# HiromasaYamanishi/furusato_recommend

Hardware: AMD Instinct MI355X
Metric: BPR positive-edges/sec (LightGCN-3 d=64, 1000000 x 100000 / 20000000 edges) (higher is better)
Workload: dtype f32; 1 GPU; C2: LightGCN 3-layer d=64, synthetic 1000000 users x 100000 items / 20000000 edges (uniform); users=1000000, items=100000, edges=20000000, graph=uniform, dim=64, layers=3, bpr_batch_per_rank=2048, global_batch=2048, ranks=1, parallelism=dp1 (user-sharded, RCCL none gradient exchange)

## Files before the change

### furusato_recommend_amd/_lib.py

```python
from __future__ import annotations

import ctypes
import os
from ctypes import (POINTER, Structure, c_float, c_int, c_int32, c_int64,
                    c_size_t, c_uint64, c_void_p, c_char_p)

import torch

_HERE = os.path.dirname(os.path.abspath(__file__))
LIB_PATH = os.environ.get("MIREC_LIB") or os.path.join(_HERE, "libmirec.so")

MIREC_OK = 0
ERR_WORKSPACE = 4
ERR_RANGE = 5
IN_PRESCALED, IN_RAW, IN_SPARSE, IN_NONE = 0, 1, 2, 3
SUPPORTED_DIMS = (4, 8, 16, 32, 64, 128, 256)


class MirecError(RuntimeError):
    pass


class CSR(Structure):
    _fields_ = [
# ... 93 lines not shown
    "mirec_csr_long_rows": (c_int, [c_void_p, c_int64, c_int32, POINTER(c_int64),
                                    POINTER(c_int64), c_void_p, c_void_p, c_void_p,
                                    c_void_p]),
    "mirec_propagate": (c_int, [POINTER(CSR), POINTER(Prop), c_void_p]),
    "mirec_propagate_sweep": (c_int, [POINTER(CSR), POINTER(Prop), POINTER(Sweep), c_void_p]),
    "mirec_sweep_sizeof": (c_size_t, []),
    "mirec_sweep_shape": (c_int, [c_int64, c_int32, c_int32, POINTER(c_int32),
                                  POINTER(c_int32)]),
    "mirec_sweep_build": (c_int, [c_void_p, c_void_p, c_int64, c_int64, c_int64, c_int32,
                                  c_int32, c_void_p, c_void_p]),
    "mirec_sweep_groups": (c_int, [c_int32]),
    "mirec_sweep_wave_sizeof": (c_size_t, []),
    "mirec_sweep_wave_build": (c_int, [c_void_p, c_void_p, c_int64, c_int64, c_int64, c_int64,
                                       c_int32, c_void_p, c_void_p, c_int64, POINTER(c_int64)]),
    "mirec_sweep_wave_pack": (c_int, [c_void_p, c_int64, c_int64, c_int64, c_int32, c_void_p,
                                      POINTER(c_int32)]),
    "mirec_propagate_sweep_wave": (c_int, [POINTER(CSR), POINTER(Prop), POINTER(SweepWave),
                                           POINTER(SweepWave), c_void_p]),
    "mirec_sweep_pace_sizeof": (c_size_t, []),
    "mirec_sweep_pace_ws_bytes": (c_size_t, []),
    "mirec_propagate_sweep_wave_paced": (c_int, [POINTER(CSR), POINTER(Prop), POINTER(SweepWave),
                                                 POINTER(SweepWave), POINTER(SweepPace),
                                                 c_void_p]),
    "mirec_sweep_wave_stamp": (c_int, [POINTER(CSR), POINTER(Prop), POINTER(SweepWave), c_void_p,
                                       c_int64, c_void_p, c_void_p]),
    "mirec_drop_sizeof": (c_size_t, []),
    "mirec_propagate_drop": (c_int, [POINTER(CSR), POINTER(Prop), POINTER(Drop), c_void_p]),
    "mirec_edge_keep_mask": (c_int, [c_void_p, c_void_p, c_int64, c_uint64, c_float, c_int32,
                                     c_void_p]),
    "mirec_edge_dot": (c_int, [POINTER(CSR), c_void_p, c_void_p, c_int32, c_void_p, c_void_p]),
    "mirec_prescale": (c_int, [c_void_p, c_void_p, c_int64, c_int32, c_void_p, c_void_p]),
    "mirec_shard_pack": (c_int, [c_void_p, c_int64, c_int32, c_int32, c_int32, c_int64, c_int64,
                                 c_void_p, c_void_p]),
    "mirec_shard_unpack": (c_int, [c_void_p, c_int64, c_int32, c_int32, c_int32, c_int64,
                                   c_int64, c_void_p, c_void_p, c_void_p, c_void_p]),
    "mirec_frontier": (c_int, [POINTER(CSR), c_void_p, c_int64, c_void_p, c_void_p, c_void_p,
                               c_int64, c_int64, c_void_p, c_void_p, c_void_p, c_void_p,
                               c_void_p, c_int32, c_void_p]),
    "mirec_seed_bits_sizeof": (c_size_t, []),
    "mirec_frontier_bits": (c_int, [POINTER(CSR), c_void_p, c_int64, c_void_p, c_void_p, c_void_p,
                                    c_int64, c_int64, c_void_p, c_void_p, c_void_p, c_void_p,
                                    c_void_p, c_int32, POINTER(SeedBits), c_void_p]),
    "mirec_propagate_seeded": (c_int, [POINTER(CSR), POINTER(Prop), POINTER(SeedBits), c_void_p]),
    "mirec_mask_compact_pair": (c_int, [c_void_p, c_void_p, c_void_p, c_int64, c_void_p, c_void_p,
                                        c_void_p, c_void_p, c_void_p, c_void_p]),
    "mirec_small_sort_workspace": (c_int, [c_int64, POINTER(c_size_t)]),
# ... 346 lines not shown
```

### furusato_recommend_amd/csrc/prop.hip

```cpp
#include <mutex>
#include <set>
#include <type_traits>
#include <utility>

#include "common.h"

namespace mirec {

struct PropK {
  const int64_t *rowptr;
  const int32_t *col;
  const float *dinv;
  int64_t n_rows;
  int64_t n_seg;
  const int32_t *seg_row;
  const int64_t *seg_beg;
  int32_t split;
  const float *x_in;
  const int32_t *slot;
  const float *seed_in;
  const float *seed;
  const float *addend;
  const float *seed2;
  float divisor;
// ... 662 lines not shown
constexpr int kPaceMaxNaps = 8;
constexpr int kPaceMaxNapUnits = 16;
constexpr int kXccIdReg = 20 | (3 << 11);

struct SweepAuxK {
  unsigned *ws;
  int32_t lead;
  int32_t every;
  int32_t nap;
  long long *stamps;
  int32_t *meta;
};

__device__ __forceinline__ unsigned pace_read(const unsigned *p) {
  unsigned v;
  asm volatile("s_load_dword %0, %1, 0x0 glc\n\ts_waitcnt lgkmcnt(0)"
               : "=&s"(v)
               : "s"(p)
               : "memory");
  return v;
}

template <int D, int U, bool SCALED, int AUX = kAuxNone, bool PACKED = false,
          bool STREAM = false>
__device__ __forceinline__ void sweep_wave_work(const PropK &a, const SweepWaveK &s,
                                                const SweepAuxK &x = SweepAuxK{}) {
  constexpr int LPR = D / 4;
  constexpr int G = 64 / LPR;
  constexpr int NB = 64 / (U * G);
  static_assert(G == 4 && U * G == MIREC_SWEEP_BATCH && kSweepThreads / 64 == MIREC_SWEEP_WAVES,
                "the host layout's steps, batches and waves");
  extern __shared__ float4 sweep_acc[];
  const int lane = threadIdx.x & 63;
  const int sub = lane % LPR;
  const int g = lane / LPR;
  const int wid = __builtin_amdgcn_readfirstlane(threadIdx.x >> 6);
  using Slot = typename std::conditional<PACKED, unsigned, long long>::type;
  const Slot *slots = reinterpret_cast<const Slot *>(s.slot);
  [[maybe_unused]] const int col_bits = 32 - s.row_bits;
  const Slot kPadRow = PACKED ? (Slot)(~0u << col_bits) : (Slot)0xffffffff00000000ull;
  const int64_t last = s.n_slots - 1;
  int adv = 0, told = 0, due = 0;
  unsigned *pace_reg = nullptr, *pace_sum = nullptr;
  if constexpr (AUX == kAuxPace) {
    const int label = (int)__builtin_amdgcn_s_getreg(kXccIdReg) & (kPaceLabels - 1);
    pace_reg = x.ws + (2 * label) * kPaceLineWords;
    pace_sum = pace_reg + kPaceLineWords;
    due = x.every;
    if (wid == 0 && lane == 0)
      (void)__hip_atomic_fetch_add(pace_reg, 1u, __ATOMIC_RELAXED, __HIP_MEMORY_SCOPE_AGENT);
  }
  auto pace = [&]() {
    if constexpr (AUX == kAuxPace) {
      if (wid != 0) return;
      ++adv;
      if (--due != 0) return;
      due = x.every;
      if (lane == 0)
        (void)__hip_atomic_fetch_add(pace_sum, (unsigned)(adv - told), __ATOMIC_RELAXED,
                                     __HIP_MEMORY_SCOPE_AGENT);
      told = adv;
#pragma unroll 1
      for (int i = 0; i < kPaceMaxNaps; ++i) {
        const long long sum = pace_read(pace_sum), reg = pace_read(pace_reg);
// ... 4 lines not shown
    }
  };
  [[maybe_unused]] long long *stamp_lds = nullptr;
  if constexpr (AUX == kAuxStamp)
    stamp_lds = reinterpret_cast<long long *>(sweep_acc + (int64_t)s.tile_rows * LPR);
  auto stamp = [&](int i) {
    if constexpr (AUX == kAuxStamp) {
      if (wid == 0 && lane == 0) stamp_lds[i] = (long long)wall_clock64();
    }
  };
#pragma unroll 1
  for (int tile = blockIdx.x; tile < s.n_tiles; tile += gridDim.x) {
    stamp(0);
    const int64_t tile_row0 = (int64_t)tile * s.tile_rows;
    const int tile_len = (int)min((int64_t)s.tile_rows, s.n_rows - tile_row0);
    const int lr0 = min(wid * s.wave_rows, tile_len);
    const int lr1 = min(lr0 + s.wave_rows, tile_len);
    for (int lr = lr0 + g; lr < lr1; lr += G) sweep_acc[lr * LPR + sub] = f4_zero();
    int64_t pos = s.wptr[(int64_t)tile * MIREC_SWEEP_WAVES + wid];
    const int64_t end = s.wptr[(int64_t)tile * MIREC_SWEEP_WAVES + wid + 1];
    const int n_batches = __builtin_amdgcn_readfirstlane((int)((end - pos) / (U * G)));
    Slot cur = __builtin_nontemporal_load(slots + min(pos + lane, last));
    if (lane >= n_batches * (U * G)) cur |= kPadRow;
    int band = 0;
    int64_t hi = s.src0 + s.band_rows;
    float4 pv[U];
    int pr[U];
#pragma unroll
    for (int u = 0; u < U; ++u) {
      pv[u] = f4_zero();
      pr[u] = -1;
    }
#pragma unroll 1
    for (int b0 = 0; b0 < n_batches; b0 += NB) {
      Slot nxt = __builtin_nontemporal_load(slots + min(pos + 64 + lane, last));
      if (b0 * (U * G) + 64 + lane >= n_batches * (U * G)) nxt |= kPadRow;
      int ccol, crow;
      if constexpr (PACKED) {
        ccol = (int)s.src0 + (int)(cur & ~kPadRow);
        crow = cur >= kPadRow ? -1 : (int)(cur >> col_bits);
      } else {
        ccol = (int)(cur & 0xffffffffll);
        crow = (int)(cur >> 32);
      }
#pragma unroll
      for (int k = 0; k < NB; ++k) {
        const int nc = __builtin_amdgcn_readlane(ccol, k * U * G);
        while (b0 + k < n_batches && band + 1 < s.n_bands && (int64_t)nc >= hi) {
          pace();
          __builtin_amdgcn_s_barrier();
          ++band;
          hi += s.band_rows;
          stamp(band);
        }
        float4 v[U];
        int r[U];
#pragma unroll
        for (int u = 0; u < U; ++u) {
          const int src = k * U * G + u * G + g;
          const int j = __shfl(ccol, src);
          r[u] = __shfl(crow, src);
          v[u] = ld4(a.x_in + (int64_t)j * D + sub * 4);
        }
#pragma unroll
        for (int u = 0; u < U; ++u) {
          if (pr[u] >= 0) {
            float4 *p = &sweep_acc[pr[u] * LPR + sub];
            *p = f4_add(*p, pv[u]);
          }
        }
#pragma unroll
        for (int u = 0; u < U; ++u) {
          pv[u] = v[u];
          pr[u] = r[u];
        }
      }
      pos += 64;
      cur = nxt;
    }
    while (band + 1 < s.n_bands) {
      pace();
      __builtin_amdgcn_s_barrier();
      ++band;
      stamp(band);
    }
#pragma unroll
    for (int u = 0; u < U; ++u) {
      if (pr[u] >= 0) {
        float4 *p = &sweep_acc[pr[u] * LPR + sub];
        *p = f4_add(*p, pv[u]);
      }
    }
    for (int lr = lr0 + g; lr < lr1; lr += G)
      row_epilogue<D, SCALED, STREAM>(a, s.row0 + tile_row0 + lr, sweep_acc[lr * LPR + sub],
                                      sub);
    if constexpr (AUX == kAuxStamp) {
      stamp(s.n_bands);
      if (wid == 0) {
        long long *o = x.stamps + (int64_t)tile * (s.n_bands + 1);
        for (int b = lane; b <= s.n_bands; b += 64) o[b] = stamp_lds[b];
        if (lane == 0) {
// ... 12 lines not shown
      asm volatile("s_waitcnt vmcnt(0)" ::: "memory");
      unsigned *done = x.ws + 2 * kPaceLabels * kPaceLineWords;
      const unsigned left = __hip_atomic_fetch_add(done, 1u, __ATOMIC_RELAXED,
                                                   __HIP_MEMORY_SCOPE_AGENT);
      if (left == gridDim.x - 1) {
        for (int i = 0; i <= 2 * kPaceLabels; ++i)
          __hip_atomic_store(x.ws + i * kPaceLineWords, 0u, __ATOMIC_RELAXED,
                             __HIP_MEMORY_SCOPE_AGENT);
      }
    }
  }
}

template <int D, int U, bool SCALED, bool PACKED = false, bool STREAM = false>
__global__ __launch_bounds__(kSweepThreads) __attribute__((amdgpu_waves_per_eu(4, 4)))
MIREC_NO_PK_F32 void prop_sweep_wave_kernel(PropK a, SweepWaveK s) {
  sweep_wave_work<D, U, SCALED, kAuxNone, PACKED, STREAM>(a, s);
}

template <int D, int U, bool SCALED, int AUX, bool PACKED = false, bool STREAM = false>
__global__ __launch_bounds__(kSweepThreads) __attribute__((amdgpu_waves_per_eu(4, 4)))
MIREC_NO_PK_F32 void prop_sweep_wave_aux_kernel(PropK a, SweepWaveK s, SweepAuxK x) {
  sweep_wave_work<D, U, SCALED, AUX, PACKED, STREAM>(a, s, x);
}

using PropFn = void (*)(PropK);

template <int D, int UNROLL>
static PropFn prop_kernel_for(int mode, bool masked, bool rowmask, bool weighted, bool scaled,
                              bool dropout) {
  if (mode == MIREC_IN_SPARSE) masked = true;
  if (mode == MIREC_IN_NONE) weighted = dropout = false;
#define MIREC_PROP_CASE(MODE_W, MASKED)                               \
  case (MODE_W) * 2 + (MASKED):                                       \
    return rowmask ? prop_kernel<D, UNROLL, (MODE_W), MASKED, true>   \
                   : prop_kernel<D, UNROLL, (MODE_W), MASKED, false>;
  switch ((mode | (weighted ? kWeighted : 0) | (scaled ? kScaled : 0) |
           (dropout ? kDropout : 0)) * 2 + masked) {
    MIREC_PROP_CASE(MIREC_IN_PRESCALED | kWeighted, false)
    MIREC_PROP_CASE(MIREC_IN_PRESCALED, false)
    MIREC_PROP_CASE(MIREC_IN_PRESCALED | kWeighted, true)
    MIREC_PROP_CASE(MIREC_IN_PRESCALED, true)
    MIREC_PROP_CASE(MIREC_IN_RAW | kWeighted, false)
    MIREC_PROP_CASE(MIREC_IN_RAW, false)
    MIREC_PROP_CASE(MIREC_IN_RAW | kWeighted, true)
    MIREC_PROP_CASE(MIREC_IN_RAW, true)
// ... 145 lines not shown
      }
#pragma unroll
      for (int u = 0; u < UNROLL; ++u) {
        const float d = group_sum<LPR>(f4_dot(va[u], vb[u]));
        const float t = __shfl(d, (lane & (G - 1)) * LPR);
        if (lane >= k + u * G && lane < k + (u + 1) * G) res = t;
      }
    }
    if (lane < cnt) out[base + lane] = res;
  }
}

template <int D, int UNROLL>
static int launch_edge_dot(const mirec_csr_t *c, const float *a, const float *b, float *out,
                           hipStream_t st) {
  const int64_t waves = (c->nnz + kDotChunk - 1) / kDotChunk;
  const int64_t blocks = (waves + kWavesPerBlock - 1) / kWavesPerBlock;
  hipLaunchKernelGGL((edge_dot_kernel<D, UNROLL>), dim3((unsigned)blocks), dim3(256), 0, st,
                     c->rowptr, c->col, c->n_rows, c->nnz, a, b, out);
  MIREC_LAUNCH_CHECK();
  return MIREC_OK;
}

static bool sweep_launch_qualifies(const mirec_csr_t *c, const mirec_prop_t *p) {
  if (p->dim != 64) return false;
  if (c->val != nullptr) return false;
  if (p->in_mode != MIREC_IN_PRESCALED) return false;
  if (p->in_mask != nullptr || p->row_mask != nullptr || p->row_list != nullptr) return false;
  return c->n_seg == 0;
}

static bool sweep_qualifies(const mirec_csr_t *c, const mirec_prop_t *p, const mirec_sweep_t *sw) {
  if (sw == nullptr || !sweep_launch_qualifies(c, p)) return false;
  if (sw->gptr == nullptr || sw->ent == nullptr || sw->n_rows <= 0 || sw->n_tiles <= 0)
    return false;
  if (sw->row0 < 0 || sw->row0 + sw->n_rows != c->n_rows || sw->n_src > c->n_rows) return false;
  if (sw->tile_rows <= 0 || sw->group_rows <= 0 || sw->band_rows <= 0) return false;
  if (sw->groups <= 0 || sw->groups > kSweepThreads / (64 / 4)) return false;
  if ((int64_t)sw->groups * sw->group_rows < sw->tile_rows) return false;
  if ((int64_t)sw->n_tiles * sw->tile_rows < sw->n_rows) return false;
  if ((int64_t)sw->tile_rows * 64 * 4 > kSweepLdsDefault) return false;
  return true;
}

template <int D, int UNROLL>
static int launch_head(const mirec_csr_t *c, const PropK &k, int64_t row0, hipStream_t st) {
  mirec_csr_t head = *c;
  head.n_rows = row0;
  PropK kh = k;
  kh.n_rows = row0;
  return launch_prop<D, UNROLL>(&head, kh, 0, MIREC_IN_PRESCALED, st);
}

template <int D, int UNROLL>
static int launch_sweep(const mirec_csr_t *c, const PropK &k, const mirec_sweep_t *sw,
                        hipStream_t st) {
  SweepK s;
  s.gptr = sw->gptr;
  s.ent = reinterpret_cast<const long long *>(sw->ent);
  s.row0 = sw->row0;
  s.n_rows = sw->n_rows;
  s.tile_rows = sw->tile_rows;
  s.group_rows = sw->group_rows;
  s.groups = sw->groups;
  s.band_rows = sw->band_rows;
  s.n_bands = (int32_t)std::max<int64_t>(1, (sw->n_src + sw->band_rows - 1) / sw->band_rows);
  const size_t lds = (size_t)sw->tile_rows * D * sizeof(float);
  const auto kernel =
      k.scale_next != nullptr ? prop_sweep_kernel<D, 4, true> : prop_sweep_kernel<D, 4, false>;
  hipLaunchKernelGGL(kernel, dim3((unsigned)sw->n_tiles), dim3(kSweepThreads), lds, st, k, s);
  MIREC_LAUNCH_CHECK();
  if (sw->row0 == 0) return MIREC_OK;
  return launch_head<D, UNROLL>(c, k, sw->row0, st);
}
// ... 24 lines not shown
  MIREC_HIP(hipGetDevice(&dev));
  std::lock_guard<std::mutex> lock(mu);
  if (raised.count({kernel, dev}) != 0) return MIREC_OK;
  MIREC_HIP(hipFuncSetAttribute(kernel, hipFuncAttributeMaxDynamicSharedMemorySize,
                                kSweepLdsMax));
  raised.insert({kernel, dev});
  return MIREC_OK;
}

struct SweepStamp {
  const mirec_sweep_wave_t *layout;
  int64_t *stamps;
  int64_t stamps_len;
  int32_t *meta;
};

static int32_t sweep_wave_bands(const mirec_sweep_wave_t *w) {
  return (int32_t)std::max<int64_t>(1, (w->n_src + w->band_rows - 1) / w->band_rows);
}

template <int D>
static int launch_sweep_wave(const PropK &k, const mirec_sweep_wave_t *w, hipStream_t st,
                             const mirec_sweep_pace_t *pace = nullptr, int block = 0,
                             const SweepStamp *stamp = nullptr, bool stream = false) {
  SweepWaveK s;
  s.wptr = w->wptr;
  s.slot = reinterpret_cast<const long long *>(w->slot);
  s.n_slots = w->n_slots;
  s.row0 = w->row0;
  s.n_rows = w->n_rows;
  s.src0 = w->src0;
  s.tile_rows = w->tile_rows;
  s.wave_rows = w->wave_rows;
  s.n_tiles = w->n_tiles;
  s.band_rows = w->band_rows;
  s.n_bands = sweep_wave_bands(w);
  s.row_bits = w->row_bits;
  size_t lds = (size_t)w->tile_rows * D * sizeof(float);
  const bool scaled = k.scale_next != nullptr;
  const bool packed = w->row_bits != 0;
  stream = stream && packed && k.param != nullptr;
  if (stamp != nullptr) {
    SweepAuxK x = {};
    x.stamps = reinterpret_cast<long long *>(stamp->stamps);
    x.meta = stamp->meta;
    lds += (size_t)(s.n_bands + 1) * sizeof(long long);
    if (packed) return MIREC_ERR_ARG;
    const auto kernel = scaled ? prop_sweep_wave_aux_kernel<D, 4, true, kAuxStamp>
                               : prop_sweep_wave_aux_kernel<D, 4, false, kAuxStamp>;
    if (lds > (size_t)kSweepLdsDefault &&
        hipFuncSetAttribute(reinterpret_cast<const void *>(kernel),
                            hipFuncAttributeMaxDynamicSharedMemorySize, (int)lds) != hipSuccess)
      return MIREC_ERR_HIP;
    hipLaunchKernelGGL(kernel, dim3((unsigned)w->grid), dim3(kSweepThreads), lds, st, k, s, x);
  } else if (pace != nullptr && pace->every[block] > 0) {
    SweepAuxK x = {};
    x.ws = reinterpret_cast<unsigned *>(pace->ws) + block * kPaceRegionWords;
    x.lead = pace->lead_bands[block];
    x.every = pace->every[block];
    x.nap = pace->nap[block];
    auto kernel = scaled ? prop_sweep_wave_aux_kernel<D, 4, true, kAuxPace>
                         : prop_sweep_wave_aux_kernel<D, 4, false, kAuxPace>;
    if (packed)
      kernel = scaled ? prop_sweep_wave_aux_kernel<D, 4, true, kAuxPace, true>
                      : prop_sweep_wave_aux_kernel<D, 4, false, kAuxPace, true>;
// ... 12 lines not shown
      kernel = scaled ? prop_sweep_wave_kernel<D, 4, true, true, true>
                      : prop_sweep_wave_kernel<D, 4, false, true, true>;
    const int rc = sweep_lds_allow(reinterpret_cast<const void *>(kernel), lds);
    if (rc != MIREC_OK) return rc;
    hipLaunchKernelGGL(kernel, dim3((unsigned)w->grid), dim3(kSweepThreads), lds, st, k, s);
  }
  MIREC_LAUNCH_CHECK();
  return MIREC_OK;
}

}

extern "C" int mirec_sweep_groups(int32_t dim) {
  return dim == 64 ? mirec::kSweepThreads / (64 / 4) : 0;
}

namespace mirec {

static int propagate(const mirec_csr_t *c, const mirec_prop_t *p, const mirec_sweep_t *sw,
                     const mirec_sweep_wave_t *wi, const mirec_sweep_wave_t *wu,
                     mirec_stream_t stream, const mirec_drop_t *drop = nullptr,
                     const mirec_sweep_pace_t *pace = nullptr,
                     const SweepStamp *stamp = nullptr,
                     const mirec_seed_bits_t *seeded = nullptr) {
  MIREC_CHECK_ARG(c != nullptr && p != nullptr);
  if (pace != nullptr) {
    MIREC_CHECK_ARG(pace->ws != nullptr);
    for (int b = 0; b < 2; ++b)
      MIREC_CHECK_ARG(pace->every[b] >= 0 && pace->lead_bands[b] >= 0 && pace->nap[b] >= 0 &&
                      pace->nap[b] <= kPaceMaxNapUnits);
  }
  MIREC_CHECK_ARG(c->rowptr != nullptr && c->dinv != nullptr && c->n_rows >= 0);
  MIREC_CHECK_ARG(c->nnz == 0 || c->col != nullptr);
  if (!dim_supported(p->dim)) return MIREC_ERR_DIM;
  MIREC_CHECK_ARG(p->in_mode >= 0 && p->in_mode <= 3);
  if (p->in_mode == MIREC_IN_SPARSE)
    MIREC_CHECK_ARG(p->slot != nullptr && p->seed_in != nullptr);
  else if (p->in_mode != MIREC_IN_NONE)
    MIREC_CHECK_ARG(p->x_in != nullptr);
  MIREC_CHECK_ARG(p->in_mode != MIREC_IN_NONE || p->in_mask == nullptr);
  MIREC_CHECK_ARG((p->seed == nullptr && p->seed2 == nullptr) || p->slot != nullptr);
  MIREC_CHECK_ARG(p->param == nullptr || (p->exp_avg != nullptr && p->exp_avg_sq != nullptr));
  MIREC_CHECK_ARG(p->divisor != 0.f);
  MIREC_CHECK_ARG(p->row_list == nullptr ||
                  (p->row_count != nullptr && p->row_list_cap >= 0 && p->row_mask != nullptr));
  MIREC_CHECK_ARG(p->wide_list == nullptr || (p->row_list != nullptr && p->wide_count != nullptr));
  if (c->n_seg > 0) {
    MIREC_CHECK_ARG(c->split > 0 && c->seg_row && c->seg_beg && c->long_rows && c->long_segptr);
// ... 53 lines not shown
    k.drop_scale = 1.f / drop->keep_prob;
  }
  const int64_t cap = p->row_list_cap;
  hipStream_t st = reinterpret_cast<hipStream_t>(stream);
  const bool nt = p->adam_stream != 0 && p->param != nullptr;
  if (stamp != nullptr) {
    const mirec_sweep_wave_t *w = stamp->layout;
    MIREC_CHECK_ARG(w != nullptr && stamp->stamps != nullptr && stamp->meta != nullptr);
    MIREC_CHECK_ARG(sweep_launch_qualifies(c, p) && w->row0 >= 0 && w->n_rows > 0 &&
                    w->row0 + w->n_rows <= c->n_rows &&
                    sweep_wave_valid(c, w, w->row0, w->n_rows));
    MIREC_CHECK_ARG(stamp->stamps_len >= (int64_t)w->n_tiles * (sweep_wave_bands(w) + 1));
    return launch_sweep_wave<64>(k, w, st, nullptr, 0, stamp);
  }
  if (sweep_qualifies(c, p, sw)) return launch_sweep<64, 4>(c, k, sw, st);
  if (wi != nullptr && sweep_launch_qualifies(c, p) &&
      sweep_wave_valid(c, wi, wi->row0, c->n_rows - wi->row0)) {
    const int rc = launch_sweep_wave<64>(k, wi, st, pace, 0, nullptr, nt);
    if (rc != MIREC_OK || wi->row0 == 0) return rc;
    if (sweep_wave_valid(c, wu, 0, wi->row0))
      return launch_sweep_wave<64>(k, wu, st, pace, 1, nullptr, nt);
    return launch_head<64, 4>(c, k, wi->row0, st);
  }
  if (seeded != nullptr) {
    switch (p->dim) {
      case 4: return launch_seeded<4, 1>(k, seeded, c->nnz, cap, st);
      case 8: return launch_seeded<8, 1>(k, seeded, c->nnz, cap, st);
      case 16: return launch_seeded<16, 1>(k, seeded, c->nnz, cap, st);
      case 32: return launch_seeded<32, 2>(k, seeded, c->nnz, cap, st);
      case 64: return launch_seeded<64, 4>(k, seeded, c->nnz, cap, st);
      case 128: return launch_seeded<128, 4>(k, seeded, c->nnz, cap, st);
      case 256: return launch_seeded<256, 4>(k, seeded, c->nnz, cap, st);
    }
    return MIREC_ERR_DIM;
  }
  switch (p->dim) {
    case 4: return launch_prop<4, 1>(c, k, cap, p->in_mode, st, dropout);
    case 8: return launch_prop<8, 1>(c, k, cap, p->in_mode, st, dropout);
    case 16: return launch_prop<16, 1>(c, k, cap, p->in_mode, st, dropout);
    case 32: return launch_prop<32, 2>(c, k, cap, p->in_mode, st, dropout);
    case 64: return launch_prop<64, 4>(c, k, cap, p->in_mode, st, dropout, nt);
    case 128: return launch_prop<128, 4>(c, k, cap, p->in_mode, st, dropout);
    case 256: return launch_prop<256, 8>(c, k, cap, p->in_mode, st, dropout);
  }
  return MIREC_ERR_DIM;
}
// ... 9 lines not shown
                                     const mirec_sweep_t *sw, mirec_stream_t stream) {
  return mirec::propagate(c, p, sw, nullptr, nullptr, stream);
}

extern "C" int mirec_propagate_sweep_wave(const mirec_csr_t *c, const mirec_prop_t *p,
                                          const mirec_sweep_wave_t *items,
                                          const mirec_sweep_wave_t *users,
                                          mirec_stream_t stream) {
  return mirec::propagate(c, p, nullptr, items, users, stream);
}

extern "C" size_t mirec_sweep_pace_sizeof(void) { return sizeof(mirec_sweep_pace_t); }

extern "C" size_t mirec_sweep_pace_ws_bytes(void) {
  return 2 * (size_t)mirec::kPaceRegionWords * sizeof(unsigned);
}

extern "C" int mirec_propagate_sweep_wave_paced(const mirec_csr_t *c, const mirec_prop_t *p,
                                                const mirec_sweep_wave_t *items,
                                                const mirec_sweep_wave_t *users,
                                                const mirec_sweep_pace_t *pace,
                                                mirec_stream_t stream) {
  return mirec::propagate(c, p, nullptr, items, users, stream, nullptr, pace);
}

extern "C" int mirec_sweep_wave_stamp(const mirec_csr_t *c, const mirec_prop_t *p,
                                      const mirec_sweep_wave_t *layout, int64_t *stamps,
                                      int64_t stamps_len, int32_t *meta, mirec_stream_t stream) {
  const mirec::SweepStamp s = {layout, stamps, stamps_len, meta};
  return mirec::propagate(c, p, nullptr, nullptr, nullptr, stream, nullptr, nullptr, &s);
}

extern "C" size_t mirec_drop_sizeof(void) { return sizeof(mirec_drop_t); }

extern "C" int mirec_propagate_drop(const mirec_csr_t *c, const mirec_prop_t *p,
                                    const mirec_drop_t *drop, mirec_stream_t stream) {
  return mirec::propagate(c, p, nullptr, nullptr, nullptr, stream, drop);
}

extern "C" int mirec_propagate_seeded(const mirec_csr_t *c, const mirec_prop_t *p,
                                      const mirec_seed_bits_t *filter, mirec_stream_t stream) {
  using namespace mirec;
  MIREC_CHECK_ARG(c != nullptr && p != nullptr);
  const bool shape = filter != nullptr && p->in_mode == MIREC_IN_SPARSE &&
                     p->row_list != nullptr && p->in_mask == nullptr && c->val == nullptr &&
                     c->n_seg == 0 && c->nnz > 0 && p->scale_src == nullptr &&
// ... 62 lines not shown
```

### furusato_recommend_amd/engine.py

```python
from __future__ import annotations

import ctypes
import math
import os

import torch

from . import _lib
from ._lib import (IN_NONE, IN_PRESCALED, IN_RAW, IN_SPARSE, Prop, adam_hparams,
                   check, lib, ptr)
from .graph import Graph

SWEEP_FORM = "wave"
SWEEP_USERS = True
LAYER_SUM_ROWS = "self"
SWEEP_PACE = {"items": (8, 16, 16), "users": (4, 4, 16)}
SEEDED_FIRST = True
ADAM_STREAM = True
SEEDED_LDS_BYTES = 16 * 1024


def seed_bit_layout(n0: int, n1: int, budget: int):
    def words(n, s):
        return -(-(-(-n // (1 << s))) // 32)

    def fit(n, share):
        s = 0
        while s < 31 and words(n, s) > 1 and 4 * words(n, s) > share:
            s += 1
        return s
    n = (int(n0), int(n1))
    small = 0 if n[0] <= n[1] else 1
    shift, w = [0, 0], [0, 0]
    shift[small] = fit(n[small], int(budget) * 7 // 8)
    w[small] = words(n[small], shift[small])
    shift[1 - small] = fit(n[1 - small], int(budget) - 4 * w[small])
    w[1 - small] = words(n[1 - small], shift[1 - small])
    w[1] += -(w[0] + w[1]) % 4
    return tuple(shift), tuple(w)


# ... 202 lines not shown
        self._bm = torch.zeros(2 * words + (sum(self._bit_cap) + 3) // 4 * 4, **i32)
        self.bm_self, self.bm_hop = self._bm[:words], self._bm[words:2 * words]
        self._seed_bits_mem = self._bm[2 * words:]
        B3 = max((2 + self.n_neg) * self.max_batch, 2 * self.max_batch + self.n_shared)
        self.self_list = torch.zeros(B3, **i32)
        self.self_count = torch.zeros(1, **i32)
        self._self_cap = 0
        cap = N if self.prune else 1
        self.s_lists = (torch.zeros(cap, **i32), torch.zeros(cap, **i32))
        self.hop_lists = (torch.zeros(cap, **i32), torch.zeros(cap, **i32))
        self.list_counts = torch.zeros(4, **i32)
        self.use_hop_list = True
        self.reuse_prescaled = True
        self.layer_sum_rows = LAYER_SUM_ROWS
        self.use_sweep = True
        self._group_sizes = (None, None, None)
        self._wave_sizes = {"items": (None, None), "users": (None, None), "max_grid": None}
        self.sweep_wave = self.sweep_wave_users = None
        self._sweep_form, self._sweep_users = SWEEP_FORM, SWEEP_USERS
        self._sweep_packed = None
        self.adam_stream = ADAM_STREAM
        self.sweep_pace = SWEEP_PACE
        self._pace_ws = None
        self._wave_layouts()
        self.sparse_filter = "auto"
        self.seeded_first = SEEDED_FIRST
        self._seeded_lds_bytes = SEEDED_LDS_BYTES
        self._seed_bits = None
        self._bits_ready = False
        self._masks_ready = False
        self.narrow_max = 64
        self.seed_p = torch.empty(B3, D, **f32)
        self.seed_e = torch.empty(B3, D, **f32)
        self.coef = torch.empty(self.n_neg * self.max_batch, **f32)
        self.coef_pos = self.g_u = None
        self._shared = None
        self.softplus = torch.empty(self.max_batch, **f32)
        self.reg = torch.empty(self.max_batch, **f32)
        self.keys = torch.empty(B3, **i32)
        self.vals = torch.empty(B3, **i32)
        self.keys_sorted = torch.empty(B3, **i32)
        self.loss = torch.zeros(1, **f32)
        self.partial = graph.partial_buffer(D)
        self._ws = None
        self._ws_bytes = 0
        self._ensure_ws(self.max_batch)
# ... 42 lines not shown
            self._ws = torch.empty(nb.value, dtype=torch.uint8, device=self.g.device)
            self._ws_bytes = nb.value

    def _ensure_ssm_shared(self, batch: int, m: int):
        if self._shared is None:
            dev, B, M = self.g.device, self.max_batch, self.n_shared
            f32 = dict(dtype=torch.float32, device=dev)
            self._shared = dict(coef=torch.empty(B * M, **f32), coef_pos=torch.empty(B, **f32),
                                g=torch.empty(B + M, self.dim, **f32),
                                reg=torch.empty(M, **f32),
                                mask=torch.empty(B * M, dtype=torch.uint8, device=dev))
        nb = ctypes.c_size_t(0)
        check(lib.mirec_ssm_shared_seed_workspace(batch, m, self.g.n_nodes, ctypes.byref(nb)),
              "ssm_shared_seed_workspace")
        if nb.value > self._ws_bytes:
            self._ws = torch.empty(nb.value, dtype=torch.uint8, device=self.g.device)
            self._ws_bytes = nb.value
        return self._shared

    def _prop(self, *, in_mode, x_in=None, seed_in=None, seed=None, addend=None, seed2=None,
              divisor=1.0, out=None, xs_out=None, adam=None, param=None, graph=None,
              row_mask=None, in_mask=None, row_list=None, row_count=None, row_list_cap=0,
              out_mask=None, wide_list=None, wide_count=None, direction="fwd", stamp=None,
              seeded=False):
        g = graph or self.g
        p = Prop()
        if g.scale_src is not None:
            a, b = g.scale_src.data_ptr(), g.scale_dst.data_ptr()
            if direction == "fwd":
                p.scale_src, p.scale_dst, p.scale_next = a, b, a
            elif direction in ("bwd", "bwd_last"):
                p.scale_src, p.scale_dst = b, a
                p.scale_next = a if direction == "bwd_last" else b
            else:
                raise ValueError(f"direction: 'fwd', 'bwd' or 'bwd_last', got {direction!r}")
        p.dim = self.dim
        p.in_mode = in_mode
        p.x_in = ptr(x_in)
        p.slot = self.slot.data_ptr() if (seed_in is not None or seed is not None
                                          or seed2 is not None) else None
        p.seed_in = ptr(seed_in)
        p.seed = ptr(seed)
        p.addend = ptr(addend)
        p.seed2 = ptr(seed2)
        p.divisor = float(divisor)
        p.out = ptr(out)
        p.xs_out = ptr(xs_out)
# ... 20 lines not shown
            s, e = torch.cuda.Event(enable_timing=True), torch.cuda.Event(enable_timing=True)
            s.record()
        on = self.use_sweep and g is self.g
        if stamp is not None:
            lay, stamps, meta = stamp
            check(lib.mirec_sweep_wave_stamp(g.csr_ptr(), ctypes.byref(p), lay.ptr(),
                                             stamps.data_ptr(), stamps.numel(), meta.data_ptr(),
                                             _lib.stream_handle()), "sweep_wave_stamp")
        elif self._drop is not None:
            if direction not in ("fwd", "bwd", "bwd_last"):
                raise ValueError(f"direction: 'fwd', 'bwd' or 'bwd_last', got {direction!r}")
            drop = _lib.Drop(keep_prob=self._drop[0], transposed=int(direction != "fwd"),
                             seed=self._drop[1])
            check(lib.mirec_propagate_drop(g.csr_ptr(), ctypes.byref(p), ctypes.byref(drop),
                                           _lib.stream_handle()), "propagate_drop")
        elif seeded:
            p.in_mask = None
            check(lib.mirec_propagate_seeded(g.csr_ptr(), ctypes.byref(p),
                                             ctypes.byref(self._seed_bits_struct()),
                                             _lib.stream_handle()), "propagate_seeded")
        elif on and self._sweep_form == "wave":
            wi, wu = self.sweep_wave, self.sweep_wave_users if self._sweep_users else None
            pace = self._pace_struct()
            check(lib.mirec_propagate_sweep_wave_paced(
                g.csr_ptr(), ctypes.byref(p), wi.ptr() if wi is not None else None,
                wu.ptr() if wu is not None else None,
                ctypes.byref(pace) if pace is not None else None, _lib.stream_handle()),
                "propagate")
        else:
            sw = self.sweep if on else None
            check(lib.mirec_propagate_sweep(g.csr_ptr(), ctypes.byref(p),
                                            sw.ptr() if sw is not None else None,
                                            _lib.stream_handle()), "propagate")
        if ev is not None:
            e.record()
            kind = (in_mode, in_mask is not None, row_mask is not None, out_mask is not None)
            ev.append((s, e, kind, self.launch_bytes(p, g)))

    def _pace_struct(self):
        sp = self.sweep_pace
        if sp is None:
            return None
        if self._pace_ws is None:
            self._pace_ws = torch.zeros(int(lib.mirec_sweep_pace_ws_bytes()) // 4,
                                        dtype=torch.int32, device=self.g.device)
        pace = _lib.SweepPace(ws=self._pace_ws.data_ptr())
        for b, block in enumerate(("items", "users")):
            lead, every, nap = sp.get(block) or (0, 0, 0)
            pace.lead_bands[b], pace.every[b], pace.nap[b] = int(lead), int(every), int(nap)
        return pace
# ... 53 lines not shown
                                              self._wide_bits().data_ptr(), g.n_nodes,
                                              self.s_lists[0].data_ptr(),
                                              self.s_lists[1].data_ptr(),
                                              self.hop_lists[0].data_ptr(),
                                              self.hop_lists[1].data_ptr(),
                                              self.list_counts.data_ptr(), _lib.stream_handle()),
                  "mask_compact_pair")
        self._masks_ready = True

    def set_sweep_sizes(self, tile_rows: int | None = None, group_rows: int | None = None,
                        band_rows: int | None = None, *, wave_items=None, wave_users=None,
                        max_grid: int | None = None):
        self._group_sizes = (tile_rows, group_rows, band_rows)
        self._wave_sizes = {"items": tuple(wave_items or (tile_rows, band_rows)),
                            "users": tuple(wave_users or (None, None)), "max_grid": max_grid}
        self.sweep_wave = self.sweep_wave_users = None
        self._wave_layouts()

    @property
    def sweep(self):
        return self.g.sweep_layout(self.dim, *self._group_sizes)

    def _wave_layouts(self):
        if self._sweep_form != "wave":
            return
        ws = self._wave_sizes
        if self.sweep_wave is None:
            self.sweep_wave = self.g.sweep_wave_layout(self.dim, "items", *ws["items"],
                                                       max_grid=ws["max_grid"],
                                                       packed=self._sweep_packed)
        if self._sweep_users and self.sweep_wave is not None and self.sweep_wave_users is None:
            self.sweep_wave_users = self.g.sweep_wave_layout(self.dim, "users", *ws["users"],
                                                             max_grid=ws["max_grid"],
                                                             packed=self._sweep_packed)

    @property
    def sweep_packed(self):
        return self._sweep_packed

    @sweep_packed.setter
    def sweep_packed(self, on):
        self._sweep_packed = None if on is None else bool(on)
        self.sweep_wave = self.sweep_wave_users = None
        self._wave_layouts()

    @property
    def sweep_user_tile(self):
        return self._wave_sizes["users"][0]

    @sweep_user_tile.setter
    def sweep_user_tile(self, rows):
        self._wave_sizes["users"] = (rows, self._wave_sizes["users"][1])
        self.sweep_wave_users = None
        self._wave_layouts()

    @property
    def sweep_form(self) -> str:
        return self._sweep_form

    @sweep_form.setter
    def sweep_form(self, form: str):
        if form not in ("wave", "group"):
            raise ValueError(f"sweep_form: 'wave' or 'group', got {form!r}")
        self._sweep_form = form
        self._wave_layouts()

    @property
    def sweep_users(self) -> bool:
        return self._sweep_users

    @sweep_users.setter
    def sweep_users(self, on: bool):
        self._sweep_users = bool(on)
        self._wave_layouts()

    def _wide_bits(self) -> torch.Tensor:
        key = int(self.narrow_max)
        wb = getattr(self, "_wide_bits_cache", None)
        if wb is not None and wb[0] == key:
            return wb[1]
        g = self.g
        rp = g.rowptr
        n = g.n_nodes
        wide = (rp[1:n + 1] - rp[:n]) > key
        words = (n + 31) // 32
        bits = torch.zeros(words * 32, dtype=torch.int64, device=wide.device)
        bits[:n] = wide.to(torch.int64)
# ... 345 lines not shown

        def last_layer(**kw):
            for c, rows in enumerate(chunks):
                self._prop(**kw, **final, **(rows or {}))
                if on_chunk is not None:
                    on_chunk(c)
        if L == 0:
            last_layer(in_mode=IN_NONE, seed=seed_p)
        else:
            for l in range(L - 1, -1, -1):
                first = l == L - 1
                if first:
                    rows = self._hop_rows() if (self.prune and l > 0) else {}
                    if self.sparse_filter == "dense":
                        kw = dict(in_mode=IN_PRESCALED, x_in=self._dense_seeds(seed_p, 0),
                                  in_mask=self.bm_self, **rows)
                    else:
                        kw = dict(in_mode=IN_SPARSE, seed_in=seed_p,
                                  in_mask=self._sparse_filter(), **rows)
                        if l > 0 and self._bits_ready and self._seeded_ok():
                            kw["seeded"] = True
                else:
                    kw = dict(in_mode=IN_PRESCALED, x_in=self.xs[(L - 2 - l) % 2],
                              in_mask=self.bm_hop if (self.prune and l == L - 2) else None)
                kw["seed"] = seed_p
                if l == 0:
                    last_layer(**kw)
                else:
                    kw.update(xs_out=self.xs[(L - 1 - l) % 2])
                    self._prop(**kw, direction="bwd")
        if self.sparse_filter == "dense" and L > 0:
            self._dense_seeds(seed_p, 1)
        check(lib.mirec_bpr_seed_reset(self.slot.data_ptr(), keys_sorted.data_ptr(), n_keys,
                                       _lib.stream_handle()), "bpr_seed_reset")
        self._seeds = None
        self._masks_ready = self._bits_ready = False
        self._x0s_token = self._token(emb) if (adam is not None and L > 0 and last_rows is None
                                               and self.reuse_prescaled) else None

    def adam_step(self, param: torch.Tensor, grad: torch.Tensor, adam: AdamState):
        _note_raw_write()
        self._acc_full = None
        hp = adam.next_hparams()
        check(lib.mirec_adam_dense(param.data_ptr(), grad.data_ptr(), adam.exp_avg.data_ptr(),
                                   adam.exp_avg_sq.data_ptr(), param.numel(), ctypes.byref(hp),
                                   _lib.stream_handle()), "adam_dense")

# ... 175 lines not shown
```

### include/mirec.h

```cpp
#ifndef MIREC_H
#define MIREC_H

#include <stddef.h>
#include <stdint.h>

#ifdef __cplusplus
extern "C" {
#endif

#define MIREC_ABI_VERSION 1

enum mirec_status {
  MIREC_OK = 0,
  MIREC_ERR_ARG = 1,
  MIREC_ERR_DIM = 2,
  MIREC_ERR_HIP = 3,
  MIREC_ERR_WORKSPACE = 4,
  MIREC_ERR_RANGE = 5
};

typedef void *mirec_stream_t;

const char *mirec_strerror(int code);
int mirec_abi_version(void);
// ... 170 lines not shown

int mirec_sweep_wave_pack(const int64_t *slot8, int64_t n_slots, int64_t src0, int64_t n_src,
                          int32_t tile_rows, uint32_t *slot4, int32_t *row_bits);

int mirec_propagate_sweep_wave(const mirec_csr_t *csr, const mirec_prop_t *p,
                               const mirec_sweep_wave_t *items,
                               const mirec_sweep_wave_t *users, mirec_stream_t stream);

typedef struct mirec_sweep_pace {
  void *ws;
  int32_t lead_bands[2];
  int32_t every[2];
  int32_t nap[2];
} mirec_sweep_pace_t;

size_t mirec_sweep_pace_sizeof(void);
size_t mirec_sweep_pace_ws_bytes(void);

int mirec_propagate_sweep_wave_paced(const mirec_csr_t *csr, const mirec_prop_t *p,
                                     const mirec_sweep_wave_t *items,
                                     const mirec_sweep_wave_t *users,
                                     const mirec_sweep_pace_t *pace, mirec_stream_t stream);

int mirec_sweep_wave_stamp(const mirec_csr_t *csr, const mirec_prop_t *p,
                           const mirec_sweep_wave_t *layout, int64_t *stamps,
                           int64_t stamps_len, int32_t *meta, mirec_stream_t stream);

int mirec_edge_dot(const mirec_csr_t *csr, const float *a, const float *b,
                   int32_t dim, float *out, mirec_stream_t stream);

int mirec_prescale(const float *x, const float *dinv, int64_t n_rows,
                   int32_t dim, float *out, mirec_stream_t stream);

int mirec_shard_pack(const float *table, int64_t n_rows, int32_t dim, int32_t world,
                     int32_t rank, int64_t slot0, int64_t n_slots, float *stage_rank,
                     mirec_stream_t stream);
int mirec_shard_unpack(const float *stage, int64_t n_rows, int32_t dim, int32_t world,
                       int32_t rank, int64_t slot0, int64_t n_slots, const float *dinv,
                       float *table, float *x0s, mirec_stream_t stream);

int mirec_frontier(const mirec_csr_t *csr, const int32_t *keys, int64_t n_keys,
                   const int32_t *users, const int32_t *pos, const int32_t *neg,
                   int64_t batch, int64_t n_users, uint8_t *bm_self,
                   uint8_t *bm_hop, int32_t *self_list, int32_t *self_count,
                   int32_t *zero_counts, int32_t n_zero_counts, mirec_stream_t stream);

// ... 554 lines not shown
```

Measured before the change: 608,400 positive-edges/s.

## Route pruned backward hop with input mask through the wave sweep kernel

```diff
diff --git a/furusato_recommend_amd/_lib.py b/furusato_recommend_amd/_lib.py
--- a/furusato_recommend_amd/_lib.py
+++ b/furusato_recommend_amd/_lib.py
@@ -139,6 +139,9 @@
     "mirec_propagate_sweep_wave_paced": (c_int, [POINTER(CSR), POINTER(Prop), POINTER(SweepWave),
                                                  POINTER(SweepWave), POINTER(SweepPace),
                                                  c_void_p]),
+    "mirec_propagate_sweep_wave_masked": (c_int, [POINTER(CSR), POINTER(Prop),
+                                                  POINTER(SweepWave), POINTER(SweepWave),
+                                                  POINTER(SweepPace), c_int32, c_void_p]),
     "mirec_sweep_wave_stamp": (c_int, [POINTER(CSR), POINTER(Prop), POINTER(SweepWave), c_void_p,
                                        c_int64, c_void_p, c_void_p]),
     "mirec_drop_sizeof": (c_size_t, []),
diff --git a/furusato_recommend_amd/csrc/prop.hip b/furusato_recommend_amd/csrc/prop.hip
--- a/furusato_recommend_amd/csrc/prop.hip
+++ b/furusato_recommend_amd/csrc/prop.hip
@@ -708,7 +708,7 @@
 }
 
 template <int D, int U, bool SCALED, int AUX = kAuxNone, bool PACKED = false,
-          bool STREAM = false>
+          bool STREAM = false, bool INMASK = false>
 __device__ __forceinline__ void sweep_wave_work(const PropK &a, const SweepWaveK &s,
                                                 const SweepAuxK &x = SweepAuxK{}) {
   constexpr int LPR = D / 4;
@@ -716,6 +716,8 @@
   constexpr int NB = 64 / (U * G);
   static_assert(G == 4 && U * G == MIREC_SWEEP_BATCH && kSweepThreads / 64 == MIREC_SWEEP_WAVES,
                 "the host layout's steps, batches and waves");
+  static_assert(!INMASK || (!SCALED && !STREAM && AUX != kAuxStamp && NB >= 3),
+                "the masked forms a step uses");
   extern __shared__ float4 sweep_acc[];
   const int lane = threadIdx.x & 63;
   const int sub = lane % LPR;
@@ -726,6 +728,10 @@
   [[maybe_unused]] const int col_bits = 32 - s.row_bits;
   const Slot kPadRow = PACKED ? (Slot)(~0u << col_bits) : (Slot)0xffffffff00000000ull;
   const int64_t last = s.n_slots - 1;
+  [[maybe_unused]] auto slot_col = [&](Slot v) -> int64_t {
+    if constexpr (PACKED) return s.src0 + (int64_t)(v & ~kPadRow);
+    return (int64_t)(v & 0xffffffffll);
+  };
   int adv = 0, told = 0, due = 0;
   unsigned *pace_reg = nullptr, *pace_sum = nullptr;
   if constexpr (AUX == kAuxPace) {
@@ -776,6 +782,11 @@
     const int n_batches = __builtin_amdgcn_readfirstlane((int)((end - pos) / (U * G)));
     Slot cur = __builtin_nontemporal_load(slots + min(pos + lane, last));
     if (lane >= n_batches * (U * G)) cur |= kPadRow;
+    [[maybe_unused]] int cmask = 1, nmask = 1;
+    if constexpr (INMASK) {
+      cmask = a.in_mask[slot_col(cur)];
+      asm volatile("" : "+v"(cmask));
+    }
     int band = 0;
     int64_t hi = s.src0 + s.band_rows;
     float4 pv[U];
@@ -797,6 +808,13 @@
         ccol = (int)(cur & 0xffffffffll);
         crow = (int)(cur >> 32);
       }
+      int lcol = ccol;
+      if constexpr (INMASK) {
+        if (cmask == 0) {
+          crow = -1;
+          lcol = (int)s.src0;
+        }
+      }
 #pragma unroll
       for (int k = 0; k < NB; ++k) {
         const int nc = __builtin_amdgcn_readlane(ccol, k * U * G);
@@ -807,12 +825,15 @@
           hi += s.band_rows;
           stamp(band);
         }
+        if constexpr (INMASK) {
+          if (k == 2) nmask = a.in_mask[slot_col(nxt)];
+        }
         float4 v[U];
         int r[U];
 #pragma unroll
         for (int u = 0; u < U; ++u) {
           const int src = k * U * G + u * G + g;
-          const int j = __shfl(ccol, src);
+          const int j = __shfl(lcol, src);
           r[u] = __shfl(crow, src);
           v[u] = ld4(a.x_in + (int64_t)j * D + sub * 4);
         }
@@ -831,6 +852,10 @@
       }
       pos += 64;
       cur = nxt;
+      if constexpr (INMASK) {
+        asm volatile("" : "+v"(nmask));
+        cmask = nmask;
+      }
     }
     while (band + 1 < s.n_bands) {
       pace();
@@ -889,6 +914,18 @@
 __global__ __launch_bounds__(kSweepThreads) __attribute__((amdgpu_waves_per_eu(4, 4)))
 MIREC_NO_PK_F32 void prop_sweep_wave_aux_kernel(PropK a, SweepWaveK s, SweepAuxK x) {
   sweep_wave_work<D, U, SCALED, AUX, PACKED, STREAM>(a, s, x);
+}
+
+template <int D, int U, bool PACKED>
+__global__ __launch_bounds__(kSweepThreads) __attribute__((amdgpu_waves_per_eu(4, 4)))
+MIREC_NO_PK_F32 void prop_sweep_wave_masked_kernel(PropK a, SweepWaveK s) {
+  sweep_wave_work<D, U, false, kAuxNone, PACKED, false, true>(a, s);
+}
+
+template <int D, int U, int AUX, bool PACKED>
+__global__ __launch_bounds__(kSweepThreads) __attribute__((amdgpu_waves_per_eu(4, 4)))
+MIREC_NO_PK_F32 void prop_sweep_wave_masked_aux_kernel(PropK a, SweepWaveK s, SweepAuxK x) {
+  sweep_wave_work<D, U, false, AUX, PACKED, false, true>(a, s, x);
 }
 
 using PropFn = void (*)(PropK);
@@ -1080,11 +1117,13 @@
   return MIREC_OK;
 }
 
-static bool sweep_launch_qualifies(const mirec_csr_t *c, const mirec_prop_t *p) {
+static bool sweep_launch_qualifies(const mirec_csr_t *c, const mirec_prop_t *p,
+                                   bool in_mask_ok = false) {
   if (p->dim != 64) return false;
   if (c->val != nullptr) return false;
   if (p->in_mode != MIREC_IN_PRESCALED) return false;
-  if (p->in_mask != nullptr || p->row_mask != nullptr || p->row_list != nullptr) return false;
+  if (p->in_mask != nullptr && !in_mask_ok) return false;
+  if (p->row_mask != nullptr || p->row_list != nullptr) return false;
   return c->n_seg == 0;
 }
 
@@ -1105,9 +1144,29 @@
 static int launch_head(const mirec_csr_t *c, const PropK &k, int64_t row0, hipStream_t st) {
   mirec_csr_t head = *c;
   head.n_rows = row0;
+  head.n_long = 0;
   PropK kh = k;
   kh.n_rows = row0;
   return launch_prop<D, UNROLL>(&head, kh, 0, MIREC_IN_PRESCALED, st);
+}
+
+template <int D, int UNROLL>
+static int launch_tail(const mirec_csr_t *c, const PropK &k, int64_t row0, hipStream_t st) {
+  mirec_csr_t tail = *c;
+  tail.n_rows = c->n_rows - row0;
+  if (c->n_seg != 0 || c->n_long != 0) return MIREC_ERR_ARG;
+  PropK kt = k;
+  kt.n_rows = tail.n_rows;
+  kt.rowptr += row0;
+  kt.dinv += row0;
+  if (kt.slot != nullptr) kt.slot += row0;
+  if (kt.out_mask != nullptr) kt.out_mask += row0;
+  const int64_t off = row0 * D;
+  if (kt.out != nullptr) kt.out += off;
+  if (kt.xs_out != nullptr) kt.xs_out += off;
+  if (kt.addend != nullptr) kt.addend += off;
+  if (kt.param != nullptr) kt.param += off, kt.m += off, kt.v += off;
+  return launch_prop<D, UNROLL>(&tail, kt, 0, MIREC_IN_PRESCALED, st);
 }
 
 template <int D, int UNROLL>
@@ -1178,7 +1237,8 @@
 template <int D>
 static int launch_sweep_wave(const PropK &k, const mirec_sweep_wave_t *w, hipStream_t st,
                              const mirec_sweep_pace_t *pace = nullptr, int block = 0,
-                             const SweepStamp *stamp = nullptr, bool stream = false) {
+                             const SweepStamp *stamp = nullptr, bool stream = false,
+                             bool masked = false) {
   SweepWaveK s;
   s.wptr = w->wptr;
   s.slot = reinterpret_cast<const long long *>(w->slot);
@@ -1196,7 +1256,26 @@
   const bool scaled = k.scale_next != nullptr;
   const bool packed = w->row_bits != 0;
   stream = stream && packed && k.param != nullptr;
-  if (stamp != nullptr) {
+  if (masked && (scaled || stamp != nullptr || k.in_mask == nullptr))
+    return MIREC_ERR_ARG;
+  if (masked && pace != nullptr && pace->every[block] > 0) {
+    SweepAuxK x = {};
+    x.ws = reinterpret_cast<unsigned *>(pace->ws) + block * kPaceRegionWords;
+    x.lead = pace->lead_bands[block];
+    x.every = pace->every[block];
+    x.nap = pace->nap[block];
+    const auto kernel = packed ? prop_sweep_wave_masked_aux_kernel<D, 4, kAuxPace, true>
+                               : prop_sweep_wave_masked_aux_kernel<D, 4, kAuxPace, false>;
+    const int rc = sweep_lds_allow(reinterpret_cast<const void *>(kernel), lds);
+    if (rc != MIREC_OK) return rc;
+    hipLaunchKernelGGL(kernel, dim3((unsigned)w->grid), dim3(kSweepThreads), lds, st, k, s, x);
+  } else if (masked) {
+    const auto kernel = packed ? prop_sweep_wave_masked_kernel<D, 4, true>
+                               : prop_sweep_wave_masked_kernel<D, 4, false>;
+    const int rc = sweep_lds_allow(reinterpret_cast<const void *>(kernel), lds);
+    if (rc != MIREC_OK) return rc;
+    hipLaunchKernelGGL(kernel, dim3((unsigned)w->grid), dim3(kSweepThreads), lds, st, k, s);
+  } else if (stamp != nullptr) {
     SweepAuxK x = {};
     x.stamps = reinterpret_cast<long long *>(stamp->stamps);
     x.meta = stamp->meta;
@@ -1255,8 +1334,9 @@
                      mirec_stream_t stream, const mirec_drop_t *drop = nullptr,
                      const mirec_sweep_pace_t *pace = nullptr,
                      const SweepStamp *stamp = nullptr,
-                     const mirec_seed_bits_t *seeded = nullptr) {
+                     const mirec_seed_bits_t *seeded = nullptr, int32_t masked_blocks = 0) {
   MIREC_CHECK_ARG(c != nullptr && p != nullptr);
+  MIREC_CHECK_ARG((masked_blocks & ~(MIREC_SWEEP_MASKED_ITEMS | MIREC_SWEEP_MASKED_USERS)) == 0);
   if (pace != nullptr) {
     MIREC_CHECK_ARG(pace->ws != nullptr);
     for (int b = 0; b < 2; ++b)
@@ -1356,6 +1436,20 @@
       return launch_sweep_wave<64>(k, wu, st, pace, 1, nullptr, nt);
     return launch_head<64, 4>(c, k, wi->row0, st);
   }
+  if (masked_blocks != 0 && p->in_mask != nullptr && !scaled && wi != nullptr &&
+      sweep_launch_qualifies(c, p, true) &&
+      sweep_wave_valid(c, wi, wi->row0, c->n_rows - wi->row0)) {
+    const bool mi = (masked_blocks & MIREC_SWEEP_MASKED_ITEMS) != 0;
+    const bool mu = (masked_blocks & MIREC_SWEEP_MASKED_USERS) != 0 && wi->row0 > 0 &&
+                    sweep_wave_valid(c, wu, 0, wi->row0);
+    if (mi || mu) {
+      const int rc = mi ? launch_sweep_wave<64>(k, wi, st, pace, 0, nullptr, false, true)
+                        : launch_tail<64, 4>(c, k, wi->row0, st);
+      if (rc != MIREC_OK || wi->row0 == 0) return rc;
+      return mu ? launch_sweep_wave<64>(k, wu, st, pace, 1, nullptr, false, true)
+                : launch_head<64, 4>(c, k, wi->row0, st);
+    }
+  }
   if (seeded != nullptr) {
     switch (p->dim) {
       case 4: return launch_seeded<4, 1>(k, seeded, c->nnz, cap, st);
@@ -1411,6 +1505,15 @@
                                                 const mirec_sweep_pace_t *pace,
                                                 mirec_stream_t stream) {
   return mirec::propagate(c, p, nullptr, items, users, stream, nullptr, pace);
+}
+
+extern "C" int mirec_propagate_sweep_wave_masked(const mirec_csr_t *c, const mirec_prop_t *p,
+                                                 const mirec_sweep_wave_t *items,
+                                                 const mirec_sweep_wave_t *users,
+                                                 const mirec_sweep_pace_t *pace,
+                                                 int32_t blocks, mirec_stream_t stream) {
+  return mirec::propagate(c, p, nullptr, items, users, stream, nullptr, pace, nullptr, nullptr,
+                          blocks);
 }
 
 extern "C" int mirec_sweep_wave_stamp(const mirec_csr_t *c, const mirec_prop_t *p,
diff --git a/furusato_recommend_amd/engine.py b/furusato_recommend_amd/engine.py
--- a/furusato_recommend_amd/engine.py
+++ b/furusato_recommend_amd/engine.py
@@ -17,6 +17,8 @@
 SWEEP_PACE = {"items": (8, 16, 16), "users": (4, 4, 16)}
 SEEDED_FIRST = True
 ADAM_STREAM = True
+SWEEP_INMASK = "items"
+_INMASK_BLOCKS = {"off": 0, "items": 1, "users": 2, "both": 3}
 SEEDED_LDS_BYTES = 16 * 1024
 
 
@@ -265,6 +267,7 @@
         self.adam_stream = ADAM_STREAM
         self.sweep_pace = SWEEP_PACE
         self._pace_ws = None
+        self._sweep_inmask = SWEEP_INMASK
         self._wave_layouts()
         self.sparse_filter = "auto"
         self.seeded_first = SEEDED_FIRST
@@ -353,7 +356,7 @@
               divisor=1.0, out=None, xs_out=None, adam=None, param=None, graph=None,
               row_mask=None, in_mask=None, row_list=None, row_count=None, row_list_cap=0,
               out_mask=None, wide_list=None, wide_count=None, direction="fwd", stamp=None,
-              seeded=False):
+              seeded=False, inmask_sweep=False):
         g = graph or self.g
         p = Prop()
         if g.scale_src is not None:
@@ -420,10 +423,22 @@
         elif on and self._sweep_form == "wave":
             wi, wu = self.sweep_wave, self.sweep_wave_users if self._sweep_users else None
             pace = self._pace_struct()
-            check(lib.mirec_propagate_sweep_wave_paced(
-                g.csr_ptr(), ctypes.byref(p), wi.ptr() if wi is not None else None,
-                wu.ptr() if wu is not None else None,
-                ctypes.byref(pace) if pace is not None else None, _lib.stream_handle()),
+            args = (g.csr_ptr(), ctypes.byref(p), wi.ptr() if wi is not None else None,
+                    wu.ptr() if wu is not None else None,
+                    ctypes.byref(pace) if pace is not None else None)
+            blocks = _INMASK_BLOCKS[self._sweep_inmask] if inmask_sweep else 0
+            if blocks and in_mask is not None:
+                check(lib.mirec_propagate_sweep_wave_masked(*args, blocks, _lib.stream_handle()),
+                      "propagate")
+            else:
+                check(lib.mirec_propagate_sweep_wave_paced(*args, _lib.stream_handle()),
+                      "propagate")
+        elif (on and inmask_sweep and in_mask is not None and self.sweep_wave is not None
+              and _INMASK_BLOCKS[self._sweep_inmask] & 1):
+            pace = self._pace_struct()
+            check(lib.mirec_propagate_sweep_wave_masked(
+                g.csr_ptr(), ctypes.byref(p), self.sweep_wave.ptr(), None,
+                ctypes.byref(pace) if pace is not None else None, 1, _lib.stream_handle()),
                 "propagate")
         else:
             sw = self.sweep if on else None
@@ -523,14 +538,15 @@
         return self.g.sweep_layout(self.dim, *self._group_sizes)
 
     def _wave_layouts(self):
-        if self._sweep_form != "wave":
+        if self._sweep_form != "wave" and not (_INMASK_BLOCKS[self._sweep_inmask] & 1):
             return
         ws = self._wave_sizes
         if self.sweep_wave is None:
             self.sweep_wave = self.g.sweep_wave_layout(self.dim, "items", *ws["items"],
                                                        max_grid=ws["max_grid"],
                                                        packed=self._sweep_packed)
-        if self._sweep_users and self.sweep_wave is not None and self.sweep_wave_users is None:
+        if self._sweep_form == "wave" and self._sweep_users and self.sweep_wave is not None \
+                and self.sweep_wave_users is None:
             self.sweep_wave_users = self.g.sweep_wave_layout(self.dim, "users", *ws["users"],
                                                              max_grid=ws["max_grid"],
                                                              packed=self._sweep_packed)
@@ -564,6 +580,17 @@
         if form not in ("wave", "group"):
             raise ValueError(f"sweep_form: 'wave' or 'group', got {form!r}")
         self._sweep_form = form
+        self._wave_layouts()
+
+    @property
+    def sweep_inmask(self) -> str:
+        return self._sweep_inmask
+
+    @sweep_inmask.setter
+    def sweep_inmask(self, blocks: str):
+        if blocks not in _INMASK_BLOCKS:
+            raise ValueError(f"sweep_inmask: 'off', 'items', 'users' or 'both', got {blocks!r}")
+        self._sweep_inmask = blocks
         self._wave_layouts()
 
     @property
@@ -955,7 +982,8 @@
                             kw["seeded"] = True
                 else:
                     kw = dict(in_mode=IN_PRESCALED, x_in=self.xs[(L - 2 - l) % 2],
-                              in_mask=self.bm_hop if (self.prune and l == L - 2) else None)
+                              in_mask=self.bm_hop if (self.prune and l == L - 2) else None,
+                              inmask_sweep=self.prune and l == L - 2)
                 kw["seed"] = seed_p
                 if l == 0:
                     last_layer(**kw)
diff --git a/include/mirec.h b/include/mirec.h
--- a/include/mirec.h
+++ b/include/mirec.h
@@ -216,6 +216,14 @@
                                      const mirec_sweep_wave_t *users,
                                      const mirec_sweep_pace_t *pace, mirec_stream_t stream);
 
+#define MIREC_SWEEP_MASKED_ITEMS 1
+#define MIREC_SWEEP_MASKED_USERS 2
+int mirec_propagate_sweep_wave_masked(const mirec_csr_t *csr, const mirec_prop_t *p,
+                                      const mirec_sweep_wave_t *items,
+                                      const mirec_sweep_wave_t *users,
+                                      const mirec_sweep_pace_t *pace, int32_t blocks,
+                                      mirec_stream_t stream);
+
 int mirec_sweep_wave_stamp(const mirec_csr_t *csr, const mirec_prop_t *p,
                            const mirec_sweep_wave_t *layout, int64_t *stamps,
                            int64_t stamps_len, int32_t *meta, mirec_stream_t stream);
```

New measurement: 623,500 positive-edges/s (median of 6 runs). 1.02x the previous value.
